# hzheng40/irbfn

Measured on AMD Instinct MI355X. Metric: RBF-net evals/s (B queries x N centres), forward, higher is better.
Workload: dtype f32 (distances and Phi x W on f16 MFMA: exact fixed-point heads + float tails, hi/lo operand pairs; f32 accumulate)

## Files before the change

### irbfn_amd/csrc/common.h

```cpp
#pragma once

#include <hip/hip_runtime.h>
#include <stdint.h>

#include "irbfn_hip.h"

namespace irbfn {

constexpr int kWave = 64;
constexpr int kMaxSplit = 8;
constexpr int kMaxD = 8;
constexpr int kRedBlocks = 256;
constexpr int kSeedBlocksMax = 1024;

enum BasisClass : int { BC_GAUSS = 0, BC_IQ = 1, BC_IMQ = 2, BC_GENERIC = 3 };

inline int basis_class(int basis) {
  switch (basis) {
    case IRBFN_GAUSSIAN:
    case IRBFN_GAUSSIAN_WIDE:
    case IRBFN_GAUSSIAN_WIDER: return BC_GAUSS;
    case IRBFN_INVERSE_QUADRATIC: return BC_IQ;
    case IRBFN_INVERSE_MULTIQUADRIC: return BC_IMQ;
    default: return BC_GENERIC;
// ... 82 lines not shown
  irbfn::GateTables gate() const {
    return irbfn::GateTables{gate_lo, gate_hi, gate_delta, gate_ranges, nsplit, max_ranges, n_ranges};
  }
};

namespace irbfn {
enum LaunchKind : int {
  LK_NONE = 0,
  LK_K1S,
  LK_K1R,
  LK_K1G,
  LK_K1G_WIDE,
  LK_K1H,
  LK_K1H_WIDE,
  LK_K1M,
  LK_K1,
  LK_TICK_K1G,
  LK_TICK_K1H,
  LK_TICK_K1G_WIDE,
  LK_TICK_K1H_WIDE,
  LK_K2G,
  LK_K2,
  LK_K2M,
  LK_K1G_GAMMA,
  LK_TICK_K1G_GAMMA
};

struct F16Geom {
  bool ok;
  int S, QG;
  bool pipe;
};

struct LaunchPlan {
  int kind = LK_NONE;
  int status = IRBFN_ERR_UNSUPPORTED;
  int S = 0, QG = 0;
  int terms = 3;
  bool pipe = false;
  int Q = 1, QJ = 0;
  int nw = 0;
  int QT = 1, nb = 0, cpl = 1;
  int gc = 0;
  bool gated = false;
  bool roll = false;
  bool split = false;
  int mode = -1;
  size_t lds = 0;
  int grid = 0, block = 0;
  F16Geom h = {};
};
void record_launch(irbfn_net* net, const LaunchPlan& p);

int launch_pack_all(irbfn_net* net, const float* centers, const float* log_sigs, const float* kernel, const float* bias,
                    hipStream_t s);
size_t pack_partials_bytes(const irbfn_net* net);
int launch_forward(irbfn_net* net, const float* x, float* out, int64_t B, hipStream_t s);
int launch_forward_gamma(irbfn_net* net, const float* x, const float* gamma, float* out, int64_t B, hipStream_t s);
int launch_cluster_gate(const float* x, const float* wc, const float* bc, float* logits, float* gamma, int64_t B, int D,
                        int R, hipStream_t s);
bool mfma_eligible(const irbfn_net* net);
size_t mfma_record_floats(int D, int O);
size_t mfma_lds_bytes(const irbfn_net* net, int QJ, int nw);
int launch_forward_mfma(irbfn_net* net, const LaunchPlan& p, const float* x, float* out, int64_t B, hipStream_t s);
bool f16_eligible(const irbfn_net* net);
size_t f16_image_bytes(const irbfn_net* net);
size_t f16_lds_bytes(const irbfn_net* net, int S, int QG, bool tick);
size_t f16_wide_lds_bytes(const irbfn_net* net, int SW, int QG, bool pipe);
void f16_wide_normalize(const irbfn_net* net, int* SW, int* QG, bool* pipe);
int launch_forward_f16(irbfn_net* net, const LaunchPlan& p, const float* x, float* out, int64_t B, hipStream_t s);
bool gram_eligible(const irbfn_net* net);
size_t gram_image_bytes(const irbfn_net* net);
size_t gram_header_bytes();
size_t gram_lds_bytes(int S, int QG, bool tick, bool gamma = false);
size_t gram_wide_ring_bytes(const irbfn_net* net, int SW);
size_t gram_wide_lds_bytes(const irbfn_net* net, int SW, int QG, size_t extra_red_floats);
int launch_forward_gram(irbfn_net* net, const LaunchPlan& p, const float* x, float* out, int64_t B, hipStream_t s);
int gram_gamma_cpr(const irbfn_net* net);
bool gram_gamma_eligible(const irbfn_net* net);
int gram_gamma_select(irbfn_net* net);
// ... 77 lines not shown
```

### irbfn_amd/csrc/rbf_forward.hip

```cpp
#include <math.h>
#include "rbf_forward.h"
#include "rollout_step.h"

#include <stdio.h>
#include <stdlib.h>
#include <string.h>

namespace irbfn {

int launch_forward_d3(const FwdArgs&, int, int, int, bool, bool, int, size_t, hipStream_t, int*);
int launch_forward_d4(const FwdArgs&, int, int, int, bool, bool, int, size_t, hipStream_t, int*);
int launch_forward_d7(const FwdArgs&, int, int, int, bool, bool, int, size_t, hipStream_t, int*);
int launch_forward_d8(const FwdArgs&, int, int, int, bool, bool, int, size_t, hipStream_t, int*);

static const int kCompiledOP[] = {2, 4, 5, 8, 10, 16, 32, 64, 100, 128};

int padded_O(int O) {
  for (int op : kCompiledOP)
    if (O <= op) return op;
  return -1;
}

int padded_D(int D) {
  if (D <= 3) return 3;
  if (D == 4) return 4;
  if (D <= 7) return 7;
  if (D == 8) return 8;
  return -1;
}

__global__ __launch_bounds__(64) void gate_kernel(const float* __restrict__ x, float* __restrict__ gamma,
                                                  GateTables gt, long B, int D, int R) {
  extern __shared__ float gtab[];
// ... 192 lines not shown
}

static bool gram_wide_preferred(const irbfn_net* net, int64_t B) {
  return net->gram_img && net->gram_ok && net->O > 16 && net->O <= 128 && (net->DC == 7 || net->DC == 8) && B >= 2048 && net->N >= 256;
}

static void gram_geometry(const irbfn_net* net, int64_t B, int nchunks, int* S_out, int* QG_out) {
  const long groups = (B + 31) / 32;
  int S = groups <= 512 ? 4 : (groups <= 2048 ? 2 : 1);
  while (S > 1 && nchunks / (2 * S) < 4) S /= 2;
  S = opt_or(net, IRBFN_OPT_FWD_F16_S, S);
  if (S > 7 || S > nchunks) S = 1;
  int QG = opt_or(net, IRBFN_OPT_FWD_F16_QG, (S == 1 && groups > 2048 && groups <= 3072) ? 4 : 8 / S);
  if (S * QG > 16) QG = 1;
  *S_out = S; *QG_out = QG;
}

static void gram_wide_geometry(const irbfn_net* net, int64_t B, int* SW_out, int* QG_out) {
  const int nchunks = (net->N + 31) / 32;
  const long groups = (B + 31) / 32;
  int SW = 1;
  while (SW < 4 && (groups * SW + 7) / 8 < 256) SW *= 2;
  SW = opt_or(net, IRBFN_OPT_FWD_F16_S, SW);
  if (SW != 1 && SW != 2 && SW != 4) SW = 1;
  while (SW > 1 && (gram_wide_ring_bytes(net, SW) > 160 * 1024 || nchunks / SW < 2)) SW /= 2;
  int QG = groups <= 384 ? 2 : (SW == 1 ? 4 : 8 / SW);
  QG = opt_or(net, IRBFN_OPT_FWD_F16_QG, QG);
  if (QG < 1 || SW * QG > 8) QG = 8 / SW;
  *SW_out = SW; *QG_out = QG;
}

static bool gram_slices_fit(int nchunks, int S) { return (long)nchunks * S < (1L << 31); }

static bool plan_gram(const irbfn_net* net, int64_t B, LaunchPlan* p) {
  if (!net->f16_img || !gram_eligible(net)) return false;
  int S, QG;
  size_t lds;
  if (net->O > 16) {
    if ((net->DC != 7 && net->DC != 8) || net->O > 128) return false;
    gram_wide_geometry(net, B, &S, &QG);
    lds = gram_wide_lds_bytes(net, S, QG, 0);
    p->kind = LK_K1G_WIDE;
  } else {
    gram_geometry(net, B, (net->N + 31) / 32, &S, &QG);
    if (!gram_slices_fit((net->N + 31) / 32, S)) return false;
    lds = gram_lds_bytes(S, QG, false);
    p->kind = LK_K1G;
  }
  if (lds > 160 * 1024) {
    p->kind = LK_NONE;
    return false;
  }
  p->status = IRBFN_OK;
  p->S = S; p->QG = QG; p->lds = lds;
  p->grid = (int)(((B + 31) / 32 + QG - 1) / QG); p->block = S * QG * 64;
  return true;
}

static LaunchPlan plan_forward(const irbfn_net* net, int64_t B) {
  LaunchPlan p;
  const int forced = net->opt[IRBFN_OPT_FWD_KERNEL];
  if (forced == IRBFN_FWD_AUTO && small_eligible(net, B)) {
    small_geometry(net, B, &p);
    return p;
  }
  if (forced == IRBFN_FWD_K1R || (forced == IRBFN_FWD_AUTO && sparse_preferred(net, B))) {
    p.status = sparse_geometry(net, B, false, 0, 0, &p);
    if (p.status != IRBFN_ERR_UNSUPPORTED || forced == IRBFN_FWD_K1R) return p;
  }
  if (forced == IRBFN_FWD_K1G) {
    if (net->gram_img && net->gram_ok) plan_gram(net, B, &p);
    return p;
  }
  p.h = f16_geometry(net, B);
  if (p.h.ok) {
    const bool gram = net->O > 16 ? gram_wide_preferred(net, B) : gram_preferred(net, B);
    if (forced == IRBFN_FWD_AUTO && gram && plan_gram(net, B, &p)) return p;
    if (plan_f16(net, B, &p)) return p;
  }
  if (forced == IRBFN_FWD_K1H) return p;
  if (prefer_mfma(net) && plan_mfma(net, B, &p)) return p;
  if (forced == IRBFN_FWD_K1M) return p;
  const F16Geom h = p.h;
  p = plan_qlane(net, B, net->R > 1, false);
  p.h = h;
  return p;
}

// ... 6 lines not shown
  if (!fp.h.ok || net->O > 16 || f16_terms(net) != 3) return false;
  *lds = f16_lds_bytes(net, fp.h.S, fp.h.QG, true);
  return *lds <= 64 * 1024;
}

static bool tick_through_controls(const irbfn_net* net, const LaunchPlan& fp, int64_t B) {
  return B > 64 && (prefer_mfma(net) || (fp.h.ok && net->O <= 16));
}

static LaunchPlan plan_tick(const irbfn_net* net, int mode, int64_t B, int T, bool controls) {
  const LaunchPlan fp = plan_forward(net, B);
  if (fp.status == IRBFN_ERR_HIP) return fp;
  const int forced = net->opt[IRBFN_OPT_FWD_KERNEL];
  LaunchPlan t;
  t.mode = mode; t.status = IRBFN_OK;
  auto geometry = [&](int kind, int S, int QG) {
    t.kind = kind; t.S = S; t.QG = QG;
    t.grid = (int)(((B + 31) / 32 + QG - 1) / QG); t.block = S * QG * 64;
  };
  if (tick_wide_k1h(net, fp, mode, B, T)) {
    if (fp.kind == LK_K1G_WIDE) {
      geometry(LK_TICK_K1G_WIDE, fp.S, fp.QG);
      t.lds = gram_wide_tick_lds_bytes(net, fp.S, fp.QG);
      if (t.lds <= 160 * 1024) return t;
    }
    geometry(LK_TICK_K1H_WIDE, fp.h.S, fp.h.QG);
    t.lds = f16_wide_tick_lds_bytes(net, fp.h.S, fp.h.QG);
    if (t.lds <= 160 * 1024) return t;
  }
  const bool gram_tick = fp.kind == LK_K1G && (forced != IRBFN_FWD_K1G || gram_preferred(net, B));
  if (gram_tick && net->opt[IRBFN_OPT_TICK_FUSED] != 0 && tick_narrow_compiled(net, mode, T)) {
    geometry(LK_TICK_K1G, fp.S, fp.QG);
    t.lds = gram_lds_bytes(fp.S, fp.QG, true);
    if (t.lds <= 160 * 1024) return t;
  }
  if (tick_narrow_k1h(net, fp, mode, T, &t.lds)) {
    geometry(LK_TICK_K1H, fp.h.S, fp.h.QG);
    return t;
  }
  if (fp.kind == LK_K1R) {
    LaunchPlan r;
    r.status = sparse_geometry(net, B, true, mode, T, &r);
    if (r.status != IRBFN_ERR_UNSUPPORTED) return r;
  }
  if (controls && tick_through_controls(net, fp, B)) {
    LaunchPlan f = fp;
    f.split = true;
    return f;
  }
  t = LaunchPlan();
  if (net->bclass == BC_GENERIC) return t;
  if (T * rollout_state_dim(mode) > 64) return t;
  return plan_qlane(net, B, net->R > 1, true);
}

int tick_needs_controls(const irbfn_net* net, int mode, int64_t B, int T) {
  if (B <= 64) return 0;
  const LaunchPlan fp = plan_forward(net, B);
  size_t lds;
  if (tick_wide_k1h(net, fp, mode, B, T) || tick_narrow_k1h(net, fp, mode, T, &lds)) return 0;
  return tick_through_controls(net, fp, B) ? 1 : 0;
}

void record_launch(irbfn_net* net, const LaunchPlan& p) {
  char* n = net->last_name;
  const size_t len = sizeof(net->last_name);
// ... 76 lines not shown
      break;
    }
    default: return p.status;
  }
  if (rc == IRBFN_OK) record_launch(net, p);
  return rc;
}

int launch_forward(irbfn_net* net, const float* x, float* out, int64_t B, hipStream_t s) {
  if (B == 0) return IRBFN_OK;
  return launch_planned(net, plan_forward(net, B), x, out, B, s);
}

static LaunchPlan plan_gram_gamma(const irbfn_net* net, int64_t B, bool tick, int mode) {
  LaunchPlan p;
  if (!gram_gamma_eligible(net)) return p;
  const bool packed = net->gram_img && net->f16_img && (net->R == 1 || net->gamma_packed);
  if (!packed) { p.status = IRBFN_ERR_NO_PARAMS; return p; }
  if (!net->gram_ok) return p;
  const int nchunks = net->R * gram_gamma_cpr(net);
  int S, QG;
  gram_geometry(net, B, nchunks, &S, &QG);
  const int fs = net->opt[IRBFN_OPT_FWD_F16_S];
  if (fs > 0 && fs <= 7 && S != fs) {
    S = fs;
    QG = opt_or(net, IRBFN_OPT_FWD_F16_QG, 8 / S > 0 ? 8 / S : 1);
    if (S * QG > 16) QG = 1;
  }
  p.lds = gram_lds_bytes(S, QG, tick, true);
  if (p.lds > 160 * 1024 || !gram_slices_fit(nchunks, S)) return p;
  p.kind = tick ? LK_TICK_K1G_GAMMA : LK_K1G_GAMMA; p.status = IRBFN_OK; p.mode = mode;
  p.S = S; p.QG = QG;
  p.grid = (int)(((B + 31) / 32 + QG - 1) / QG); p.block = S * QG * 64;
  return p;
}

int launch_forward_gamma(irbfn_net* net, const float* x, const float* gamma, float* out, int64_t B, hipStream_t s) {
  if (B == 0) return IRBFN_OK;
  if (net->opt[IRBFN_OPT_FWD_GAMMA_KERNEL] == IRBFN_FWDG_K1G) {
    const LaunchPlan g = plan_gram_gamma(net, B, false, -1);
    if (g.kind == LK_NONE) return g.status;
    const int rc = launch_forward_gram_gamma(net, g, x, gamma, out, B, s);
    if (rc == IRBFN_OK) record_launch(net, g);
    return rc;
  }
  const LaunchPlan p = plan_qlane(net, B, true, false);
  if (p.kind == LK_NONE) return p.status;
  FwdArgs a;
  fill_args(net, a, x, out, B);
  a.gamma_ext = gamma;
  const int rc = launch_qlane(net, p, a, s);
  if (rc == IRBFN_OK) record_launch(net, p);
  return rc;
}

static int forward_controls_only(irbfn_net* net, const float* x, const float* gamma, const int* mirror, float* controls, int64_t B,
                                 hipStream_t s) {
  if (!controls) return IRBFN_ERR_BAD_ARG;
  const int rc = gamma ? launch_forward_gamma(net, x, gamma, controls, B, s) : launch_forward(net, x, controls, B, s);
  if (rc != IRBFN_OK || !mirror) return rc;
  return launch_unmirror(controls, mirror, B, net->O, net->O / 2, s);
}

static int check_tick(const irbfn_net* net, int mode, int T) {
  if (mode != IRBFN_ROLLOUT_ST_SELECT && mode != IRBFN_ROLLOUT_ST_KS && mode != IRBFN_ROLLOUT_FULLINT &&
      mode != IRBFN_ROLLOUT_FRENET_LS)
// ... 80 lines not shown
```

### irbfn_amd/csrc/rbf_forward_gram.h

```cpp
#pragma once

#include "rbf_forward_f16_narrow.h"

namespace irbfn {

typedef _Float16 h4_t __attribute__((ext_vector_type(4)));

constexpr int kGramHeadBytes = 2 * 64 * 8;
constexpr int kGramTailBytes = 2 * 2 * 64 * 16;
constexpr int kGramOpBytes = kGramHeadBytes + kGramTailBytes;
constexpr int gram_chunk_bytes(int NT = 1) { return kGramOpBytes + NT * 2 * kF16WBytes; }
constexpr int kGramChunkBytes = gram_chunk_bytes(1);
constexpr int kGramDims = 8;
#ifndef IRBFN_GRAM_RING
#define IRBFN_GRAM_RING 5
#endif
constexpr int kGramRing = IRBFN_GRAM_RING;
#ifndef IRBFN_GRAM_WAVES
#define IRBFN_GRAM_WAVES 4
#endif

struct GramHdr {
  float r[8];
  int ex, ec, eq, ea, e2;
  int ok;
  float cabs, amax, cmax, c2max;
};

struct GramSlot { int kind, dim, p, q; };
__host__ __device__ constexpr int gram_comb_p(int m) { return m == 0 ? 0 : (m == 1 ? 1 : (m == 2 ? 0 : (m == 3 ? 2 : 1))); }
__host__ __device__ constexpr int gram_comb_q(int m) { return m == 0 ? 1 : (m == 1 ? 0 : (m == 2 ? 2 : (m == 3 ? 0 : 1))); }
__host__ __device__ constexpr GramSlot gram_head_slot(int s) {
  const int g = s >> 2, j = s & 3;
  return j < 2 ? GramSlot{1, 2 * g + j, 0, 0}
               : (j == 2 ? (g == 0 ? GramSlot{2, 0, 0, 0} : (g == 1 ? GramSlot{3, 0, 0, 0} : (g == 2 ? GramSlot{3, 0, 1, 0} : GramSlot{0, 0, 0, 0})))
                         : GramSlot{0, 0, 0, 0});
}
__host__ __device__ constexpr GramSlot gram_tail_slot(int s) {
  const int hf = s >> 5, g = (s >> 3) & 3, j = s & 7;
  const int m = hf * 3 + (j - 5);
  return j < 5 ? GramSlot{1, 2 * g + hf, gram_comb_p(j), gram_comb_q(j)}
               : (g == 0 ? (m < 5 ? GramSlot{2, 0, gram_comb_p(m), gram_comb_q(m)} : GramSlot{3, 0, 2, 0})
                         : (g == 1 && hf == 0 && j == 5 ? GramSlot{3, 0, 3, 0} : GramSlot{0, 0, 0, 0}));
}
static_assert(kGramDims == 8, "four lane groups x two coordinates");
__host__ __device__ inline int gram_T(const GramHdr& h, const GramSlot sl) {
  return sl.kind == 1 ? h.ex + h.ec - 11 * (sl.p + sl.q) : (sl.kind == 2 ? h.eq + h.ea - 11 * (sl.p + sl.q) : h.e2 - 11 * sl.p);
}
__host__ __device__ inline int gram_ax(int T) { return (T + 1) >> 1; }

template <int BC>
__host__ __device__ constexpr float gram_phi_scale() { return BC == BC_IMQ ? 128.0f : kPhiScale; }

#ifdef IRBFN_GRAM_STAMPS
__device__ unsigned long long g_gram_stamps[64];
#define IRBFN_GRAM_T() __builtin_amdgcn_s_memtime()
#define IRBFN_GRAM_PHASE(k)                                                                            \
  do {                                                                                                 \
    asm volatile("s_waitcnt vmcnt(0) lgkmcnt(0)" ::: "memory");                                        \
    if (blockIdx.x < 2 && threadIdx.x == 0) {                                                          \
      g_gram_stamps[blockIdx.x * 32 + 8 + (k)] = __builtin_amdgcn_s_memtime();                         \
      if ((k) == 0 || (k) == 6) g_gram_stamps[blockIdx.x * 32 + 16 + (k) / 6] = __builtin_amdgcn_s_memrealtime(); \
    }                                                                                                  \
  } while (0)
#else
#define IRBFN_GRAM_T() 0ull
#define IRBFN_GRAM_PHASE(k) do { } while (0)
#endif
enum GramPhase : int { GP_ENTRY = 0, GP_OPERANDS, GP_BARRIER1, GP_LOOP0, GP_LOOP1, GP_GATE, GP_STORED };

typedef float f2_t __attribute__((ext_vector_type(2)));
typedef unsigned u2_t __attribute__((ext_vector_type(2)));

__device__ __forceinline__ void split_pair_mix(float p0, float p1, unsigned& hi, unsigned& lo) {
  hi = __builtin_bit_cast(unsigned, __builtin_amdgcn_cvt_pkrtz(p0, p1));
  const float q0 = p0 * kLoGain, q1 = p1 * kLoGain;
  const float ng = -kLoGain;
  float d0, d1;
  asm("v_fma_mix_f32 %0, %1, %2, %3 op_sel:[0,0,0] op_sel_hi:[1,0,0]" : "=v"(d0) : "v"(hi), "s"(ng), "v"(q0));
  asm("v_fma_mix_f32 %0, %1, %2, %3 op_sel:[1,0,0] op_sel_hi:[1,0,0]" : "=v"(d1) : "v"(hi), "s"(ng), "v"(q1));
  lo = __builtin_bit_cast(unsigned, __builtin_amdgcn_cvt_pkrtz(d0, d1));
}

template <int BC>
__device__ __forceinline__ void trans16(const f4_t (&u)[2][2], float (&o)[16]) {
#define IRBFN_T8(OP, T)                                                                                                          \
  asm volatile(OP " %0, %8\n " OP " %1, %9\n " OP " %2, %10\n " OP " %3, %11\n " OP " %4, %12\n " OP " %5, %13\n " OP " %6, %14\n " OP     \
               " %7, %15" IRBFN_T8_TAIL##T                                                                                       \
               : "=&v"(o[8 * T]), "=&v"(o[8 * T + 1]), "=&v"(o[8 * T + 2]), "=&v"(o[8 * T + 3]), "=&v"(o[8 * T + 4]),           \
                 "=&v"(o[8 * T + 5]), "=&v"(o[8 * T + 6]), "=&v"(o[8 * T + 7])                                                   \
               : "v"(u[T][0][0]), "v"(u[T][0][1]), "v"(u[T][0][2]), "v"(u[T][0][3]), "v"(u[T][1][0]), "v"(u[T][1][1]),           \
                 "v"(u[T][1][2]), "v"(u[T][1][3]));
#define IRBFN_T8_TAIL0 ""
#define IRBFN_T8_TAIL1 "\n s_nop 7"
  if constexpr (BC == BC_GAUSS) { IRBFN_T8("v_exp_f32_e32", 0) IRBFN_T8("v_exp_f32_e32", 1) }
  else if constexpr (BC == BC_IQ) { IRBFN_T8("v_rcp_f32_e32", 0) IRBFN_T8("v_rcp_f32_e32", 1) }
  else { IRBFN_T8("v_rsq_f32_e32", 0) IRBFN_T8("v_rsq_f32_e32", 1) }
#undef IRBFN_T8
#undef IRBFN_T8_TAIL0
#undef IRBFN_T8_TAIL1
}

struct GramArgs {
  F16Args f;
  const unsigned char* __restrict__ gimg;
  const GramHdr* __restrict__ hdr;
  GateRow g0;
  int nsteps;
};

__device__ __forceinline__ void gram_parts_f(float vh, float vl, float inv, float (&n)[3]) {
  const float a = vh * inv, b = vl * inv;
  n[0] = __builtin_rintf(a * 1024.0f) * (1.0f / 1024.0f);
  const float r1 = ((a - n[0]) + b) * 2048.0f;
  n[1] = (float)(_Float16)r1;
  const float r2 = (r1 - n[1]) * 2048.0f;
  n[2] = (float)(_Float16)r2;
}

template <int DC>
__device__ __forceinline__ void gram_query_loads(const F16Args& a, const GramHdr* hp, const long (&qrow)[2], int g, float (&xv)[2][2],
                                                 float (&rv)[2]) {
#pragma unroll
  for (int c = 0; c < 2; ++c) rv[c] = hp->r[2 * g + c];
#pragma unroll
  for (int t = 0; t < 2; ++t)
#pragma unroll
    for (int c = 0; c < 2; ++c) {
      const int i = 2 * g + c;
      const bool in = i < DC && i < a.Dreal;
      const float v = a.x[qrow[t] * a.Dreal + (in ? i : 0)];
      xv[t][c] = in ? v : 0.0f;
    }
}

template <int DC>
__device__ __forceinline__ bool gram_query_operands(const F16Args& a, const GramHdr* hp, const float (&xin)[2][2], const float (&rin)[2],
                                                    int g, h4_t (&bhd)[2], h8_t (&btl)[2][2]) {
#pragma clang fp contract(off)
  static_assert(DC <= kGramDims, "eight coordinate slots");
  const int ex = hp->ex, ec = hp->ec, eq = hp->eq, ea = hp->ea, e2 = hp->e2;
// ... 149 lines not shown
```

### irbfn_amd/csrc/rbf_forward_gram.hip

```cpp
#include <hip/hip_fp16.h>
#include <stdint.h>
#include <stdio.h>
#include <stdlib.h>

#include <atomic>

#include "rbf_forward_gram_body.h"

namespace irbfn {

constexpr int kMaxDevices = 64;

template <int DC, int BC>
__global__ __launch_bounds__(1024, IRBFN_GRAM_WAVES) void rbf_fwd_f16gram(const GramArgs ga) {
  extern __shared__ __attribute__((aligned(16))) unsigned char lds[];
  gram_body<DC, BC, false>(ga, F16Roll{}, -1, lds);
}

template <int DC, int BC>
__global__ __launch_bounds__(1024, IRBFN_GRAM_WAVES) void rbf_tick_f16gram(const GramArgs ga, const F16Roll rl, const int mode) {
  extern __shared__ __attribute__((aligned(16))) unsigned char lds[];
  gram_body<DC, BC, true>(ga, rl, mode, lds);
}

static int gram_nt(const irbfn_net* net) { return (net->O + 15) / 16; }

bool gram_eligible(const irbfn_net* net) {
  return f16_eligible(net) && net->DC <= kGramDims;
}

size_t gram_image_bytes(const irbfn_net* net) {
  const int nchunks = (net->N + kF16Chunk - 1) / kF16Chunk;
  return (size_t)nchunks * gram_chunk_bytes(gram_nt(net));
}

size_t gram_header_bytes() { return sizeof(GramHdr); }

#ifdef IRBFN_GRAM_STAMPS
extern "C" int irbfn_debug_gram_stamps(unsigned long long* out64) {
  return (int)hipMemcpyFromSymbol(out64, HIP_SYMBOL(g_gram_stamps), sizeof(unsigned long long) * 64);
}
#endif

struct DynLdsSet { std::atomic<unsigned> bytes[kMaxDevices]; };
static int ensure_dyn_lds(const void* kernel, size_t lds, DynLdsSet* set) {
  if (lds <= 48 * 1024) return IRBFN_OK;
  int dev = 0;
  IRBFN_HIP_CHECK(hipGetDevice(&dev));
  if (dev >= 0 && dev < kMaxDevices && set->bytes[dev].load(std::memory_order_relaxed) >= lds) return IRBFN_OK;
  IRBFN_HIP_CHECK(hipFuncSetAttribute(kernel, hipFuncAttributeMaxDynamicSharedMemorySize, (int)lds));
  if (dev >= 0 && dev < kMaxDevices) set->bytes[dev].store((unsigned)lds, std::memory_order_relaxed);
  return IRBFN_OK;
}

template <int DC>
static int launch_gram_bc(const GramArgs& a, int bc, int grid, int block, size_t lds, hipStream_t s) {
#define IRBFN_GCASE(BCV)                                                                                      \
  case BCV: {                                                                                                 \
    auto k = rbf_fwd_f16gram<DC, BCV>;                                                                        \
    static DynLdsSet set;                                                                                     \
    if (const int rc = ensure_dyn_lds(reinterpret_cast<const void*>(k), lds, &set); rc != IRBFN_OK) return rc; \
    hipLaunchKernelGGL(k, dim3(grid), dim3(block), lds, s, a);                                                \
    break;                                                                                                    \
  }
  switch (bc) {
    IRBFN_GCASE(BC_GAUSS)
    IRBFN_GCASE(BC_IQ)
    IRBFN_GCASE(BC_IMQ)
    default: return IRBFN_ERR_UNSUPPORTED;
  }
#undef IRBFN_GCASE
  IRBFN_HIP_CHECK(hipGetLastError());
  return IRBFN_OK;
}

size_t gram_lds_bytes(int S, int QG, bool tick, bool gamma) {
  size_t ring = (size_t)S * kGramRing * kGramChunkBytes;
  if (gamma) ring += (size_t)S * QG * 128 * sizeof(float);
  else ring += (size_t)QG * 32 * sizeof(float);
  size_t red = (size_t)S * QG * 2 * 4 * 64 + (size_t)QG * 32;
  if (tick) red += (size_t)QG * 32 * (kTickNarrowCP + kTickNarrowSP);
  red *= sizeof(float);
  return ring > red ? ring : red;
}

int launch_forward_gram(irbfn_net* net, const LaunchPlan& p, const float* x, float* out, int64_t B, hipStream_t s) {
  if (p.kind == LK_K1G_WIDE) return launch_forward_gram_wide(net, p, x, out, B, s);
  GramArgs a;
  gram_fill_args(net, x, out, B, p.S, p.QG, &a);
  switch (net->DC) {
    case 3: return launch_gram_bc<3>(a, net->bclass, p.grid, p.block, p.lds, s);
    case 4: return launch_gram_bc<4>(a, net->bclass, p.grid, p.block, p.lds, s);
    case 7: return launch_gram_bc<7>(a, net->bclass, p.grid, p.block, p.lds, s);
    case 8: return launch_gram_bc<8>(a, net->bclass, p.grid, p.block, p.lds, s);
    default: return IRBFN_ERR_UNSUPPORTED;
  }
}

template <int DC>
static int launch_tick_gram_bc(const GramArgs& a, const F16Roll& rl, int mode, int bc, int grid, int block, size_t lds, hipStream_t s) {
#define IRBFN_GCASE(BCV)                                                                                      \
  case BCV: {                                                                                                 \
    auto k = rbf_tick_f16gram<DC, BCV>;                                                                       \
    static DynLdsSet set;                                                                                     \
    if (const int rc = ensure_dyn_lds(reinterpret_cast<const void*>(k), lds, &set); rc != IRBFN_OK) return rc; \
    hipLaunchKernelGGL(k, dim3(grid), dim3(block), lds, s, a, rl, mode);                                      \
    break;                                                                                                    \
  }
  switch (bc) {
    IRBFN_GCASE(BC_GAUSS)
    IRBFN_GCASE(BC_IQ)
    IRBFN_GCASE(BC_IMQ)
    default: return IRBFN_ERR_UNSUPPORTED;
  }
#undef IRBFN_GCASE
  IRBFN_HIP_CHECK(hipGetLastError());
  return IRBFN_OK;
}

int launch_tick_gram_narrow(irbfn_net* net, const LaunchPlan& p, const float* x, const int* mirror, const float* state0,
                            const DynParams& dp, float* controls, float* states, int64_t B, int T, hipStream_t s) {
  GramArgs a;
  gram_fill_args(net, x, controls, B, p.S, p.QG, &a);
  F16Roll rl;
  rl.state0 = state0; rl.states = states; rl.mirror = mirror; rl.T = T; rl.wlds = 0; rl.dp = dp;
  return net->DC == 7 ? launch_tick_gram_bc<7>(a, rl, p.mode, net->bclass, p.grid, p.block, p.lds, s)
                      : launch_tick_gram_bc<8>(a, rl, p.mode, net->bclass, p.grid, p.block, p.lds, s);
}

}
```

### irbfn_amd/csrc/rbf_forward_gram_body.h

```cpp
#pragma once

#include "rbf_forward_gram.h"

namespace irbfn {

struct GramGamma {
  const float* __restrict__ gamma;
  int R, cpr;
};

template <int DC, int BC, bool ROLL, bool GAMMA = false>
__device__ __forceinline__ void gram_body(const GramArgs& ga, const F16Roll& rl, int mode, unsigned char* lds,
                                          [[maybe_unused]] const GramGamma gm = GramGamma{nullptr, 1, 1}) {
  static_assert(DC <= kGramDims, "eight coordinate slots");
  const F16Args& a = ga.f;
  constexpr int CBL = f16_chunk_bytes(DC);
  constexpr int CB = kGramChunkBytes;
  const int tid = threadIdx.x, lane = tid & 63;
  IRBFN_GRAM_PHASE(GP_ENTRY);
  const int wave = __builtin_amdgcn_readfirstlane(tid >> 6);
  const int S = a.S, QG = a.QG;
  int slice = 0;
#pragma unroll
  for (int s2 = 1; s2 < 8; ++s2) slice += wave >= s2 * QG ? 1 : 0;
// ... 68 lines not shown
  auto gamma_stage = [&](int period) {
    if constexpr (GAMMA) {
      if (period * kGramPer >= nsteps) return;
      int l = __builtin_amdgcn_mbcnt_hi(~0u, __builtin_amdgcn_mbcnt_lo(~0u, 0u));
      asm volatile("" : "+v"(l));
      const int st = period * kGramPer + ((l >> 5) < kGramPer ? (l >> 5) : kGramPer - 1);
      int reg = (c0 + st) / gm.cpr;
      reg = reg < gm.R ? reg : gm.R - 1;
      const int ql = (l & 31) < glim ? (l & 31) : glim;
      __builtin_amdgcn_global_load_lds((gptr_t)(grow + (unsigned)(ql * gm.R + reg)), (lptr_t)(gtile + (period & 1) * 64), 4, 0, 0);
    }
  };
  [[maybe_unused]] float gcur[2] = {1.0f, 1.0f};
  auto gamma_read = [&](int i) {
    if constexpr (GAMMA) {
      const float* gp = gtile + ((i / kGramPer) & 1) * 64 + (i % kGramPer) * 32 + n;
      gcur[0] = gp[0];
      gcur[1] = gp[16];
    }
  };

  auto end_of_step = [&](int i, int b0) {
    if ((i % kGramPer) != kGramPer - 1) return;
    step_barrier();
#pragma unroll
    for (int j = 0; j < kGramPer; ++j) {
      int slot = b0 - (kGramPer - 1) + j;
      slot = slot < 0 ? slot + kGramRing : slot;
      stage(i + kGramPer + 2 + j, slot);
    }
    gamma_stage(i / kGramPer + 2);
  };

  f4_t acc[2] = {{0, 0, 0, 0}, {0, 0, 0, 0}};
  f4_t acl[2] = {{0, 0, 0, 0}, {0, 0, 0, 0}};
  auto distances = [&](const unsigned char* buf, f4_t (&u)[2][2]) { gram_distances(buf, lane, bhd, btl, u); };
  auto products = [&](float (&t16)[16], const unsigned char* buf, auto pre) {
    const h8_t bh = *reinterpret_cast<const h8_t*>(buf + kGramOpBytes + lane * 16);
    const h8_t bl = *reinterpret_cast<const h8_t*>(buf + kGramOpBytes + kF16WBytes + lane * 16);
    pre(t16);
    if constexpr (GAMMA) {
#pragma unroll
      for (int j = 0; j < 16; ++j) t16[j] *= gcur[j >> 3];
    }
#pragma unroll
    for (int t = 0; t < 2; ++t) {
      unsigned wh[4], wl[4];
#pragma unroll
      for (int jj = 0; jj < 4; ++jj) split_pair_mix(t16[t * 8 + 2 * jj], t16[t * 8 + 2 * jj + 1], wh[jj], wl[jj]);
      const h8_t ah = __builtin_bit_cast(h8_t, u4_t{wh[0], wh[1], wh[2], wh[3]});
      const h8_t al = __builtin_bit_cast(h8_t, u4_t{wl[0], wl[1], wl[2], wl[3]});
      acc[t] = __builtin_amdgcn_mfma_f32_16x16x32_f16(ah, bh, acc[t], 0, 0, 0);
      acl[t] = __builtin_amdgcn_mfma_f32_16x16x32_f16(al, bh, acl[t], 0, 0, 0);
      acl[t] = __builtin_amdgcn_mfma_f32_16x16x32_f16(ah, bl, acl[t], 0, 0, 0);
    }
  };

#pragma unroll
  for (int k = 0; k <= kGramPer; ++k) stage(k, k);
  gamma_stage(0);
  step_barrier();
  IRBFN_GRAM_PHASE(GP_BARRIER1);
#pragma unroll
  for (int k = kGramPer + 1; k < kGramRing; ++k) stage(k, k);
  gamma_stage(1);
  IRBFN_GRAM_PHASE(GP_LOOP0);
  if (!wave_bad) {
    f4_t ua[2][2], ub[2][2];
    if (na > 0) distances(ring, ua);
    asm volatile("s_nop 7\n\ts_nop 7" ::: "memory");
    int b0 = 0;
    [[maybe_unused]] unsigned long long tph[5] = {0, 0, 0, 0, 0};
    auto one_step = [&](int i, f4_t (&ucur)[2][2], f4_t (&unxt)[2][2]) {
      const int b1 = next3(b0);
      [[maybe_unused]] const unsigned long long t0 = IRBFN_GRAM_T();
      if (i + 1 < na) distances(ring + b1 * CB, unxt);
      if (i < na) {
        gamma_read(i);
        float t16[16];
        products(t16, ring + b0 * CB, [&](float (&o)[16]) { trans16<BC>(ucur, o); });
      }
      [[maybe_unused]] const unsigned long long t2 = IRBFN_GRAM_T();
      end_of_step(i, b0);
      [[maybe_unused]] const unsigned long long t4 = IRBFN_GRAM_T();
#ifdef IRBFN_GRAM_STAMPS
      tph[1] += t2 - t0; tph[2] += t4 - t2; tph[4] += 1;
#endif
      b0 = b1;
    };
    for (int i = 0; i < nsteps; i += 2) {
      one_step(i, ua, ub);
      if (i + 1 < nsteps) one_step(i + 1, ub, ua);
    }
#ifdef IRBFN_GRAM_STAMPS
    if (blockIdx.x < 2 && tid == 0)
      for (int k = 0; k < 5; ++k) g_gram_stamps[blockIdx.x * 32 + k] = tph[k];
#endif
  } else {
    int b0 = 0;
    for (int i = 0; i < nsteps; ++i) {
      if (i < na) {
        gamma_read(i);
        float t16[16];
        gram_valu_args<DC, BC, GAMMA>(a, qrow, g, reinterpret_cast<const float*>(a.img + (size_t)(c0 + i) * CBL), t16);
        products(t16, ring + b0 * CB, [&](float (&o)[16]) { trans_block<BC, 16>(o); });
      }
      end_of_step(i, b0);
      b0 = next3(b0);
    }
  }
  IRBFN_GRAM_PHASE(GP_LOOP1);
#pragma unroll
  for (int t = 0; t < 2; ++t)
#pragma unroll
    for (int r = 0; r < 4; ++r) acc[t][r] = __builtin_fmaf(acl[t][r], kLoScale, acc[t][r]);

  float gam[2] = {0.0f, 0.0f};
  if constexpr (GAMMA) {
    gam[0] = gam[1] = 1.0f;
  } else if (slice == 0) {
    gam[0] = gpark[n];
    gam[1] = gpark[16 + n];
  }
#ifdef IRBFN_GRAM_STAMPS
  asm volatile("" ::"v"(gam[0]), "v"(gam[1]));
#endif
  IRBFN_GRAM_PHASE(GP_GATE);
  narrow_epilogue<ROLL>(a, rl, mode, lds, acc, gam, S, slice, qg, q0, 1.0f / (gram_phi_scale<BC>() * kWScale));
  IRBFN_GRAM_PHASE(GP_STORED);
}

}
```

### irbfn_amd/csrc/rbf_forward_gram_gamma.hip

```cpp
#ifdef IRBFN_GRAM_STAMPS
#undef IRBFN_GRAM_STAMPS
#endif
#include <hip/hip_fp16.h>
#include <stdint.h>

#include "rbf_forward_gram_body.h"

namespace irbfn {

template <int DC, int BC>
__global__ __launch_bounds__(1024, IRBFN_GRAM_WAVES) void rbf_fwd_f16gram_gamma(const GramArgs ga, const GramGamma gm) {
  extern __shared__ __attribute__((aligned(16))) unsigned char lds[];
  gram_body<DC, BC, false, true>(ga, F16Roll{}, -1, lds, gm);
}

template <int DC, int BC>
__global__ __launch_bounds__(1024, IRBFN_GRAM_WAVES) void rbf_tick_f16gram_gamma(const GramArgs ga, const GramGamma gm, const F16Roll rl,
                                                                                 const int mode) {
  extern __shared__ __attribute__((aligned(16))) unsigned char lds[];
  gram_body<DC, BC, true, true>(ga, rl, mode, lds, gm);
}

int gram_gamma_cpr(const irbfn_net* net) { return (net->K + kF16Chunk - 1) / kF16Chunk; }

bool gram_gamma_eligible(const irbfn_net* net) {
  return net->bclass != BC_GENERIC && net->O <= 16 && (net->DC == 3 || net->DC == 4 || net->DC == 7 || net->DC == 8);
}

int gram_gamma_select(irbfn_net* net) {
  if (!gram_gamma_eligible(net) || net->R == 1 || net->gram_img) return IRBFN_OK;
  const size_t nchunks = (size_t)net->R * gram_gamma_cpr(net);
  void* bufs[5] = {nullptr, nullptr, nullptr, nullptr, nullptr};
  const size_t bytes[5] = {nchunks * f16_chunk_bytes(net->DC, 1), 128 * sizeof(float), nchunks * kGramChunkBytes, sizeof(GramHdr),
                           pack_partials_bytes(net)};
  for (int i = 0; i < 5; ++i) {
    const hipError_t e = hipMalloc(&bufs[i], bytes[i]);
    if (e != hipSuccess) {
      g_last_hip_error = (int)e;
      for (int j = 0; j < i; ++j) (void)hipFree(bufs[j]);
      return IRBFN_ERR_HIP;
    }
  }
  net->f16_img = static_cast<unsigned char*>(bufs[0]);
  net->f16_oscale = static_cast<float*>(bufs[1]);
  net->gram_img = static_cast<unsigned char*>(bufs[2]);
  net->gram_hdr = bufs[3];
  net->pack_part = static_cast<float*>(bufs[4]);
  net->gamma_packed = 0;
  return IRBFN_OK;
}

static void gamma_fill_args(const irbfn_net* net, const float* x, const float* gamma, float* out, int64_t B, int S, int QG, GramArgs* a,
                            GramGamma* gm) {
  gram_fill_args(net, x, out, B, S, QG, a);
  gm->gamma = gamma; gm->R = net->R; gm->cpr = gram_gamma_cpr(net);
  a->f.nchunks = gm->R * gm->cpr;
  a->nsteps = gram_nsteps(a->f.nchunks, S);
}

template <typename K, typename... Args>
static int launch_gg(K k, int grid, int block, size_t lds, hipStream_t s, Args... args) {
  if (lds > 48 * 1024) {
    hipError_t e = hipFuncSetAttribute(reinterpret_cast<const void*>(k), hipFuncAttributeMaxDynamicSharedMemorySize, (int)lds);
    if (e != hipSuccess) { g_last_hip_error = (int)e; return IRBFN_ERR_HIP; }
  }
  hipLaunchKernelGGL(k, dim3(grid), dim3(block), lds, s, args...);
  IRBFN_HIP_CHECK(hipGetLastError());
  return IRBFN_OK;
}

template <int DC>
static int launch_gg_fwd(const GramArgs& a, const GramGamma& gm, int bc, const LaunchPlan& p, hipStream_t s) {
  switch (bc) {
    case BC_GAUSS: return launch_gg(rbf_fwd_f16gram_gamma<DC, BC_GAUSS>, p.grid, p.block, p.lds, s, a, gm);
    case BC_IQ: return launch_gg(rbf_fwd_f16gram_gamma<DC, BC_IQ>, p.grid, p.block, p.lds, s, a, gm);
    case BC_IMQ: return launch_gg(rbf_fwd_f16gram_gamma<DC, BC_IMQ>, p.grid, p.block, p.lds, s, a, gm);
    default: return IRBFN_ERR_UNSUPPORTED;
  }
}

template <int DC>
static int launch_gg_tick(const GramArgs& a, const GramGamma& gm, const F16Roll& rl, int bc, const LaunchPlan& p, hipStream_t s) {
  switch (bc) {
    case BC_GAUSS: return launch_gg(rbf_tick_f16gram_gamma<DC, BC_GAUSS>, p.grid, p.block, p.lds, s, a, gm, rl, p.mode);
    case BC_IQ: return launch_gg(rbf_tick_f16gram_gamma<DC, BC_IQ>, p.grid, p.block, p.lds, s, a, gm, rl, p.mode);
    case BC_IMQ: return launch_gg(rbf_tick_f16gram_gamma<DC, BC_IMQ>, p.grid, p.block, p.lds, s, a, gm, rl, p.mode);
    default: return IRBFN_ERR_UNSUPPORTED;
  }
}

int launch_forward_gram_gamma(irbfn_net* net, const LaunchPlan& p, const float* x, const float* gamma, float* out, int64_t B,
                              hipStream_t s) {
  GramArgs a;
  GramGamma gm;
  gamma_fill_args(net, x, gamma, out, B, p.S, p.QG, &a, &gm);
  switch (net->DC) {
    case 3: return launch_gg_fwd<3>(a, gm, net->bclass, p, s);
    case 4: return launch_gg_fwd<4>(a, gm, net->bclass, p, s);
    case 7: return launch_gg_fwd<7>(a, gm, net->bclass, p, s);
    case 8: return launch_gg_fwd<8>(a, gm, net->bclass, p, s);
    default: return IRBFN_ERR_UNSUPPORTED;
  }
}

int launch_tick_gram_gamma(irbfn_net* net, const LaunchPlan& p, const float* x, const float* gamma, const int* mirror,
                           const float* state0, const DynParams& dp, float* controls, float* states, int64_t B, int T, hipStream_t s) {
  GramArgs a;
  GramGamma gm;
  gamma_fill_args(net, x, gamma, controls, B, p.S, p.QG, &a, &gm);
  F16Roll rl;
  rl.state0 = state0; rl.states = states; rl.mirror = mirror; rl.T = T; rl.wlds = 0; rl.dp = dp;
  return net->DC == 7 ? launch_gg_tick<7>(a, gm, rl, net->bclass, p, s) : launch_gg_tick<8>(a, gm, rl, net->bclass, p, s);
}

}
```

### irbfn_amd/csrc/rbf_forward_gram_wide.hip

```cpp
#include "rbf_forward_gram_wide.h"

namespace irbfn {

template <int DC, int BC, int NT>
__global__ __launch_bounds__(512) void rbf_fwd_f16gram_wide(const GramArgs ga) {
  extern __shared__ __attribute__((aligned(16))) unsigned char lds[];
  wide_gram_body<DC, BC, NT, -1>(ga, F16Roll{}, lds);
}

template <int DC, int NT>
static int launch_gw_bc(const GramArgs& a, int bc, int grid, int block, size_t lds, hipStream_t s) {
#define IRBFN_GWCASE(BCV)                                                                                     \
  case BCV: {                                                                                                 \
    auto k = rbf_fwd_f16gram_wide<DC, BCV, NT>;                                                                \
    if (lds > 48 * 1024) {                                                                                    \
      hipError_t e = hipFuncSetAttribute(reinterpret_cast<const void*>(k),                                    \
                                         hipFuncAttributeMaxDynamicSharedMemorySize, (int)lds);               \
      if (e != hipSuccess) { g_last_hip_error = (int)e; return IRBFN_ERR_HIP; }                               \
    }                                                                                                         \
    hipLaunchKernelGGL(k, dim3(grid), dim3(block), lds, s, a);                                                \
    break;                                                                                                    \
  }
  switch (bc) {
    IRBFN_GWCASE(BC_GAUSS)
// ... 1 lines not shown
    IRBFN_GWCASE(BC_IMQ)
    default: return IRBFN_ERR_UNSUPPORTED;
  }
#undef IRBFN_GWCASE
  IRBFN_HIP_CHECK(hipGetLastError());
  return IRBFN_OK;
}

size_t gram_wide_ring_bytes(const irbfn_net* net, int SW) { return (size_t)SW * 3 * gram_chunk_bytes((net->O + 15) / 16); }

size_t gram_wide_lds_bytes(const irbfn_net* net, int SW, int QG, size_t extra_red_floats) {
  const size_t ring = gram_wide_ring_bytes(net, SW);
  const size_t red = ((size_t)SW * QG * 2 * 4 * 64 + (size_t)QG * 32 + extra_red_floats) * sizeof(float);
  return ring > red ? ring : red;
}

int gram_nsteps(int nchunks, int S) {
  int nsteps = 0;
  for (int s2 = 0; s2 < S; ++s2) {
    const int m = (int)((long)nchunks * (s2 + 1) / S) - (int)((long)nchunks * s2 / S);
    nsteps = m > nsteps ? m : nsteps;
  }
  return nsteps;
}

void gram_fill_args(const irbfn_net* net, const float* x, float* out, int64_t B, int S, int QG, GramArgs* a) {
  const int nchunks = (net->N + kF16Chunk - 1) / kF16Chunk;
  a->f.x = x; a->f.img = net->f16_img; a->f.oscale = net->f16_oscale; a->f.bias = net->bias; a->f.out = out; a->f.gate = net->gate();
  a->f.B = (long)B; a->f.Dreal = net->D; a->f.O = net->O; a->f.nchunks = nchunks; a->f.S = S; a->f.QG = QG;
  a->gimg = net->gram_img;
  a->hdr = reinterpret_cast<const GramHdr*>(net->gram_hdr);
  a->g0 = net->gate0;
  a->nsteps = gram_nsteps(nchunks, S);
}

int launch_forward_gram_wide(irbfn_net* net, const LaunchPlan& p, const float* x, float* out, int64_t B, hipStream_t s) {
  const int NT = (net->O + 15) / 16;
  GramArgs a;
  gram_fill_args(net, x, out, B, p.S, p.QG, &a);
  int rc;
#define IRBFN_GW_NT(DCV)                                                                      \
  switch (NT) {                                                                               \
    case 2: rc = launch_gw_bc<DCV, 2>(a, net->bclass, p.grid, p.block, p.lds, s); break;      \
    case 3: rc = launch_gw_bc<DCV, 3>(a, net->bclass, p.grid, p.block, p.lds, s); break;      \
    case 4: rc = launch_gw_bc<DCV, 4>(a, net->bclass, p.grid, p.block, p.lds, s); break;      \
    case 5: rc = launch_gw_bc<DCV, 5>(a, net->bclass, p.grid, p.block, p.lds, s); break;      \
    case 6: rc = launch_gw_bc<DCV, 6>(a, net->bclass, p.grid, p.block, p.lds, s); break;      \
    case 7: rc = launch_gw_bc<DCV, 7>(a, net->bclass, p.grid, p.block, p.lds, s); break;      \
    case 8: rc = launch_gw_bc<DCV, 8>(a, net->bclass, p.grid, p.block, p.lds, s); break;      \
    default: rc = IRBFN_ERR_UNSUPPORTED;                                                      \
  }
  if (net->DC == 7) { IRBFN_GW_NT(7) } else { IRBFN_GW_NT(8) }
#undef IRBFN_GW_NT
  return rc;
}

}
```

Baseline: 853.2 million.

## Stagger co-resident gram blocks with wave priority to desynchronize phases

The host now computes how many gram blocks can share a CU, from wave count, LDS and CU count, when the grid underfills the device. It passes that count to the kernel. Blocks that do not land in hardware slot zero (read from HW_ID) raise their wave priority for the first ~3/4 of the main loop, then drop it. The aim is to keep co-resident blocks out of phase so their MFMA and memory phases overlap instead of contending. It also adds per-block timestamp instrumentation under a debug macro, and it relies on undocumented slot/priority behaviour that could cause imbalance.

```diff
diff --git a/irbfn_amd/csrc/common.h b/irbfn_amd/csrc/common.h
--- a/irbfn_amd/csrc/common.h
+++ b/irbfn_amd/csrc/common.h
@@ -138,6 +138,10 @@
   bool pipe;
 };
 
+#ifndef IRBFN_GRAM_WAVES
+#define IRBFN_GRAM_WAVES 4
+#endif
+
 struct LaunchPlan {
   int kind = LK_NONE;
   int status = IRBFN_ERR_UNSUPPORTED;
@@ -152,6 +156,7 @@
   bool roll = false;
   bool split = false;
   int mode = -1;
+  int nseat = 1;
   size_t lds = 0;
   int grid = 0, block = 0;
   F16Geom h = {};
diff --git a/irbfn_amd/csrc/rbf_forward.hip b/irbfn_amd/csrc/rbf_forward.hip
--- a/irbfn_amd/csrc/rbf_forward.hip
+++ b/irbfn_amd/csrc/rbf_forward.hip
@@ -1,4 +1,6 @@
 #include <math.h>
+
+#include <atomic>
 #include "rbf_forward.h"
 #include "rollout_step.h"
 
@@ -257,6 +259,29 @@
 
 static bool gram_slices_fit(int nchunks, int S) { return (long)nchunks * S < (1L << 31); }
 
+static int device_cus() {
+  constexpr int kDevs = 64;
+  static std::atomic<int> cus[kDevs];
+  int dev = 0, v = 0;
+  if (hipGetDevice(&dev) != hipSuccess) return 0;
+  if (dev >= 0 && dev < kDevs && (v = cus[dev].load(std::memory_order_relaxed)) > 0) return v;
+  if (hipDeviceGetAttribute(&v, hipDeviceAttributeMultiprocessorCount, dev) != hipSuccess || v <= 0) return 0;
+  if (dev >= 0 && dev < kDevs) cus[dev].store(v, std::memory_order_relaxed);
+  return v;
+}
+
+static int gram_nseat(size_t lds, int block, int grid) {
+  const int waves = block / 64;
+  if (waves < 1 || lds == 0) return 1;
+  const int by_waves = 4 * IRBFN_GRAM_WAVES / waves, by_lds = (int)((size_t)160 * 1024 / lds);
+  int n = by_waves < by_lds ? by_waves : by_lds;
+  n = n > 4 ? 4 : n;
+  const int cus = device_cus();
+  if (n <= 1 || cus <= 0 || (long)grid > (long)n * cus) return 1;
+  const int used = (grid + cus - 1) / cus;
+  return used < n ? used : n;
+}
+
 static bool plan_gram(const irbfn_net* net, int64_t B, LaunchPlan* p) {
   if (!net->f16_img || !gram_eligible(net)) return false;
   int S, QG;
@@ -279,6 +304,7 @@
   p->status = IRBFN_OK;
   p->S = S; p->QG = QG; p->lds = lds;
   p->grid = (int)(((B + 31) / 32 + QG - 1) / QG); p->block = S * QG * 64;
+  if (p->kind == LK_K1G) p->nseat = gram_nseat(lds, p->block, p->grid);
   return true;
 }
 
@@ -351,6 +377,7 @@
   if (gram_tick && net->opt[IRBFN_OPT_TICK_FUSED] != 0 && tick_narrow_compiled(net, mode, T)) {
     geometry(LK_TICK_K1G, fp.S, fp.QG);
     t.lds = gram_lds_bytes(fp.S, fp.QG, true);
+    t.nseat = gram_nseat(t.lds, t.block, t.grid);
     if (t.lds <= 160 * 1024) return t;
   }
   if (tick_narrow_k1h(net, fp, mode, T, &t.lds)) {
@@ -493,6 +520,7 @@
   p.kind = tick ? LK_TICK_K1G_GAMMA : LK_K1G_GAMMA; p.status = IRBFN_OK; p.mode = mode;
   p.S = S; p.QG = QG;
   p.grid = (int)(((B + 31) / 32 + QG - 1) / QG); p.block = S * QG * 64;
+  p.nseat = gram_nseat(p.lds, p.block, p.grid);
   return p;
 }
 
diff --git a/irbfn_amd/csrc/rbf_forward_gram.h b/irbfn_amd/csrc/rbf_forward_gram.h
--- a/irbfn_amd/csrc/rbf_forward_gram.h
+++ b/irbfn_amd/csrc/rbf_forward_gram.h
@@ -16,8 +16,8 @@
 #define IRBFN_GRAM_RING 5
 #endif
 constexpr int kGramRing = IRBFN_GRAM_RING;
-#ifndef IRBFN_GRAM_WAVES
-#define IRBFN_GRAM_WAVES 4
+#ifndef IRBFN_GRAM_FAIR
+#define IRBFN_GRAM_FAIR 1
 #endif
 
 struct GramHdr {
@@ -53,14 +53,22 @@
 __host__ __device__ constexpr float gram_phi_scale() { return BC == BC_IMQ ? 128.0f : kPhiScale; }
 
 #ifdef IRBFN_GRAM_STAMPS
+constexpr int kGramStampBlocks = 2048;
 __device__ unsigned long long g_gram_stamps[64];
+__device__ unsigned long long g_gram_blocks[kGramStampBlocks * 8];
 #define IRBFN_GRAM_T() __builtin_amdgcn_s_memtime()
+#define IRBFN_GRAM_HWREG(id) ((unsigned)__builtin_amdgcn_s_getreg((id) | (31 << 11)))
 #define IRBFN_GRAM_PHASE(k)                                                                            \
   do {                                                                                                 \
     asm volatile("s_waitcnt vmcnt(0) lgkmcnt(0)" ::: "memory");                                        \
     if (blockIdx.x < 2 && threadIdx.x == 0) {                                                          \
       g_gram_stamps[blockIdx.x * 32 + 8 + (k)] = __builtin_amdgcn_s_memtime();                         \
       if ((k) == 0 || (k) == 6) g_gram_stamps[blockIdx.x * 32 + 16 + (k) / 6] = __builtin_amdgcn_s_memrealtime(); \
+    }                                                                                                  \
+    if (((k) == 0 || (k) == 3 || (k) == 4 || (k) == 6) && blockIdx.x < kGramStampBlocks && threadIdx.x == 0) {     \
+      g_gram_blocks[blockIdx.x * 8 + ((k) == 0 ? 0 : ((k) == 6 ? 3 : (k) - 2))] = __builtin_amdgcn_s_memrealtime(); \
+      if ((k) == 0)                                                                                    \
+        g_gram_blocks[blockIdx.x * 8 + 4] = (unsigned long long)IRBFN_GRAM_HWREG(4) | (unsigned long long)IRBFN_GRAM_HWREG(20) << 32; \
     }                                                                                                  \
   } while (0)
 #else
@@ -107,6 +115,7 @@
   const GramHdr* __restrict__ hdr;
   GateRow g0;
   int nsteps;
+  int nseat;
 };
 
 __device__ __forceinline__ void gram_parts_f(float vh, float vl, float inv, float (&n)[3]) {
diff --git a/irbfn_amd/csrc/rbf_forward_gram.hip b/irbfn_amd/csrc/rbf_forward_gram.hip
--- a/irbfn_amd/csrc/rbf_forward_gram.hip
+++ b/irbfn_amd/csrc/rbf_forward_gram.hip
@@ -39,6 +39,15 @@
 #ifdef IRBFN_GRAM_STAMPS
 extern "C" int irbfn_debug_gram_stamps(unsigned long long* out64) {
   return (int)hipMemcpyFromSymbol(out64, HIP_SYMBOL(g_gram_stamps), sizeof(unsigned long long) * 64);
+}
+extern "C" int irbfn_debug_gram_blocks(unsigned long long* out64, int clear) {
+  const size_t n = sizeof(unsigned long long) * kGramStampBlocks * 8;
+  if (clear) {
+    void* p = nullptr;
+    if (const hipError_t e = hipGetSymbolAddress(&p, HIP_SYMBOL(g_gram_blocks)); e != hipSuccess) return (int)e;
+    return (int)hipMemset(p, 0, n);
+  }
+  return (int)hipMemcpyFromSymbol(out64, HIP_SYMBOL(g_gram_blocks), n);
 }
 #endif
 
@@ -88,6 +97,7 @@
   if (p.kind == LK_K1G_WIDE) return launch_forward_gram_wide(net, p, x, out, B, s);
   GramArgs a;
   gram_fill_args(net, x, out, B, p.S, p.QG, &a);
+  a.nseat = p.nseat;
   switch (net->DC) {
     case 3: return launch_gram_bc<3>(a, net->bclass, p.grid, p.block, p.lds, s);
     case 4: return launch_gram_bc<4>(a, net->bclass, p.grid, p.block, p.lds, s);
@@ -122,6 +132,7 @@
                             const DynParams& dp, float* controls, float* states, int64_t B, int T, hipStream_t s) {
   GramArgs a;
   gram_fill_args(net, x, controls, B, p.S, p.QG, &a);
+  a.nseat = p.nseat;
   F16Roll rl;
   rl.state0 = state0; rl.states = states; rl.mirror = mirror; rl.T = T; rl.wlds = 0; rl.dp = dp;
   return net->DC == 7 ? launch_tick_gram_bc<7>(a, rl, p.mode, net->bclass, p.grid, p.block, p.lds, s)
diff --git a/irbfn_amd/csrc/rbf_forward_gram_body.h b/irbfn_amd/csrc/rbf_forward_gram_body.h
--- a/irbfn_amd/csrc/rbf_forward_gram_body.h
+++ b/irbfn_amd/csrc/rbf_forward_gram_body.h
@@ -124,6 +124,15 @@
     gamma_stage(i / kGramPer + 2);
   };
 
+  bool raised = false;
+  int nflip = 0;
+  if (IRBFN_GRAM_FAIR != 0 && ga.nseat > 1) {
+    int seat = (int)(__builtin_amdgcn_s_getreg(4 | (3 << 11)) & 15u);
+    if (S * QG >= 8) seat >>= 1;
+    raised = seat > 0;
+    nflip = raised ? ((3 * nsteps) >> 2) & ~1 : 0;
+  }
+
   f4_t acc[2] = {{0, 0, 0, 0}, {0, 0, 0, 0}};
   f4_t acl[2] = {{0, 0, 0, 0}, {0, 0, 0, 0}};
   auto distances = [&](const unsigned char* buf, f4_t (&u)[2][2]) { gram_distances(buf, lane, bhd, btl, u); };
@@ -156,6 +165,7 @@
 #pragma unroll
   for (int k = kGramPer + 1; k < kGramRing; ++k) stage(k, k);
   gamma_stage(1);
+  if (raised) __builtin_amdgcn_s_setprio(1);
   IRBFN_GRAM_PHASE(GP_LOOP0);
   if (!wave_bad) {
     f4_t ua[2][2], ub[2][2];
@@ -180,9 +190,24 @@
 #endif
       b0 = b1;
     };
-    for (int i = 0; i < nsteps; i += 2) {
-      one_step(i, ua, ub);
-      if (i + 1 < nsteps) one_step(i + 1, ub, ua);
+    if constexpr (!GAMMA) {
+      int i = 0, end = nflip;
+      for (;;) {
+        for (; i < end; i += 2) {
+          one_step(i, ua, ub);
+          if (i + 1 < nsteps) one_step(i + 1, ub, ua);
+        }
+        if (end == nsteps) break;
+        if (raised) __builtin_amdgcn_s_setprio(0);
+        end = nsteps;
+      }
+    } else {
+      for (int i = 0; i < nsteps; i += 2) {
+        one_step(i, ua, ub);
+        if (i + 1 < nsteps) one_step(i + 1, ub, ua);
+        if (raised && i + 2 == nflip) __builtin_amdgcn_s_setprio(0);
+      }
+      if (raised && nflip == 0) __builtin_amdgcn_s_setprio(0);
     }
 #ifdef IRBFN_GRAM_STAMPS
     if (blockIdx.x < 2 && tid == 0)
@@ -199,7 +224,9 @@
       }
       end_of_step(i, b0);
       b0 = next3(b0);
-    }
+      if (raised && i + 1 == nflip) __builtin_amdgcn_s_setprio(0);
+    }
+    if (raised && nflip == 0) __builtin_amdgcn_s_setprio(0);
   }
   IRBFN_GRAM_PHASE(GP_LOOP1);
 #pragma unroll
diff --git a/irbfn_amd/csrc/rbf_forward_gram_gamma.hip b/irbfn_amd/csrc/rbf_forward_gram_gamma.hip
--- a/irbfn_amd/csrc/rbf_forward_gram_gamma.hip
+++ b/irbfn_amd/csrc/rbf_forward_gram_gamma.hip
@@ -50,9 +50,11 @@
   return IRBFN_OK;
 }
 
-static void gamma_fill_args(const irbfn_net* net, const float* x, const float* gamma, float* out, int64_t B, int S, int QG, GramArgs* a,
+static void gamma_fill_args(const irbfn_net* net, const float* x, const float* gamma, float* out, int64_t B, const LaunchPlan& p, GramArgs* a,
                             GramGamma* gm) {
+  const int S = p.S, QG = p.QG;
   gram_fill_args(net, x, out, B, S, QG, a);
+  a->nseat = p.nseat;
   gm->gamma = gamma; gm->R = net->R; gm->cpr = gram_gamma_cpr(net);
   a->f.nchunks = gm->R * gm->cpr;
   a->nsteps = gram_nsteps(a->f.nchunks, S);
@@ -93,7 +95,7 @@
                               hipStream_t s) {
   GramArgs a;
   GramGamma gm;
-  gamma_fill_args(net, x, gamma, out, B, p.S, p.QG, &a, &gm);
+  gamma_fill_args(net, x, gamma, out, B, p, &a, &gm);
   switch (net->DC) {
     case 3: return launch_gg_fwd<3>(a, gm, net->bclass, p, s);
     case 4: return launch_gg_fwd<4>(a, gm, net->bclass, p, s);
@@ -107,7 +109,7 @@
                            const float* state0, const DynParams& dp, float* controls, float* states, int64_t B, int T, hipStream_t s) {
   GramArgs a;
   GramGamma gm;
-  gamma_fill_args(net, x, gamma, controls, B, p.S, p.QG, &a, &gm);
+  gamma_fill_args(net, x, gamma, controls, B, p, &a, &gm);
   F16Roll rl;
   rl.state0 = state0; rl.states = states; rl.mirror = mirror; rl.T = T; rl.wlds = 0; rl.dp = dp;
   return net->DC == 7 ? launch_gg_tick<7>(a, gm, rl, net->bclass, p, s) : launch_gg_tick<8>(a, gm, rl, net->bclass, p, s);
diff --git a/irbfn_amd/csrc/rbf_forward_gram_wide.hip b/irbfn_amd/csrc/rbf_forward_gram_wide.hip
--- a/irbfn_amd/csrc/rbf_forward_gram_wide.hip
+++ b/irbfn_amd/csrc/rbf_forward_gram_wide.hip
@@ -57,6 +57,7 @@
   a->hdr = reinterpret_cast<const GramHdr*>(net->gram_hdr);
   a->g0 = net->gate0;
   a->nsteps = gram_nsteps(nchunks, S);
+  a->nseat = 1;
 }
 
 int launch_forward_gram_wide(irbfn_net* net, const LaunchPlan& p, const float* x, float* out, int64_t B, hipStream_t s) {
```

After: 891.8 million, median of 6. 1.05x the previous value.
